# jmhb0/view_neti

Measured on AMD Instinct MI355X. Metric: TI train steps/sec (SD-1.5 512^2 bs=4 per GPU), higher is better.
Workload: dtype f16; 1 GPU; learnable_mode 0, sd15 shapes, 512x512 fp16, bs=4/GPU, grad_accum 1, full train step (VAE+16xCLIP+UNet fwd/bwd+AdamW); global_batch=4, parallelism=dp1, rccl_ranks=1, hipgraph=True

## Files before the change

include/vneti.h:

```cpp
#ifndef VNETI_H
#define VNETI_H
#include <stddef.h>
#include <stdint.h>

#ifdef __cplusplus
extern "C" {
#endif

#define VNETI_ABI_VERSION 1

int vneti_version(void);
int vneti_precision(void);
int vneti_last_error(char* buf, size_t n);

typedef struct vneti_gemm_desc {
  const void* A;
  const void* B;
  void* C;
  long long lda, ldb, ldc;
  int M, N, K;
  int batch;
  long long strideA, strideB, strideC;
  const float* bias;
  const void* rowadd;
  long long ld_rowadd;
  int rows_per_group;
  const void* resid;
  long long ldr;
  float alpha;
  int act;
  int out_f32;
  int conv_mode;
  int Hi, Wi, Ci, Ho, Wo, stride, pad_t, pad_l, ups;
  long long ldx;
  int tile_hint;
  void* workspace;
  long long workspace_bytes;
  int split_k;
  const void* gate_src;
  long long ld_gate;
  int gate_act;
  void* C2;
  long long ldc2;
  int act2;
  void* gn_sums;
  int gn_hw, gn_cpg, gn_groups, gn_slots;
  int geglu;
  int conv_korder;
} vneti_gemm_desc;

int vneti_gemm_f16(const vneti_gemm_desc* d, void* stream);
int vneti_gemm_select_tile(int M, int N, int batch);
int vneti_gemm_select_split(int M, int N, int K, int batch, int tile_hint, long long workspace_bytes);

int vneti_im2col3x3_small(const void* x, int x_is_f32, long long sb, long long sc, long long sy,
                          long long sx, void* out, int Bn, int C, int Hi, int Wi, int Ho, int Wo,
                          int stride, int pad_t, int pad_l, void* stream);

int vneti_conv3x3_in(const void* x, int x_is_f32, long long sb, long long sc, long long sy, long long sx,
                     const void* w_packed, const float* bias, void* out, long long ldo, int Bn, int C, int H, int W,
                     int Co, void* gn_sums, int gn_groups, int gn_slots, void* stream);

int vneti_transpose_f16(const void* in, long long ld_in, long long stride_in, void* out,
                        long long ld_out, long long stride_out, int rows, int cols, int batch,
                        void* stream);
#define VNETI_TRANSPOSE_MAX 4
typedef struct vneti_transpose_desc {
  const void* inp;
  long long ld_in, stride_in;
  void* out;
  long long ld_out, stride_out;
  int rows, cols, batch, _pad;
} vneti_transpose_desc;
int vneti_transpose_f16_multi(const vneti_transpose_desc* descs, int n, void* stream);

long long vneti_groupnorm_ws_floats(int Bn, int HW, int C, int G);
int vneti_groupnorm_fwd(const void* x, long long ldx, void* y, long long ldy, const float* gamma,
                        const float* beta, float* mean, float* rstd, float* ws, int Bn, int HW,
                        int C, int G, float eps, int silu, void* stream);
int vneti_groupnorm_fwd_sums(const void* x, long long ldx, void* y, long long ldy, const float* gamma,
                             const float* beta, const void* sums, int slots, float* mean, float* rstd,
// ... 220 lines not shown
```

view_neti_amd/csrc/gemm8.hip:

```cpp
#include <type_traits>

#include "common.h"
#include "gemm_args.h"

namespace {

constexpr int BM = 256, NT = 512;
constexpr int HALF_BYTES = 128 * 128;
constexpr int GN_IMG = 5;

#define VN_WAIT_VM(n) asm volatile("s_waitcnt vmcnt(" #n ")" ::: "memory")
#define VN_WAIT_LGKM0() asm volatile("s_waitcnt lgkmcnt(0)" ::: "memory")

template <int BN, int EPI, bool CONV, bool HALO = false>
__global__ __launch_bounds__(NT) void gemm8_kernel(GemmArgs g) {
  static_assert(BN == 256 || BN == 128, "tile width");
  static_assert(!HALO || (BN == 128 && CONV), "the halo-patch loop exists for the 256x128 convolution tile");
  constexpr int PATCH_STRIDE = 41 * 1024;
  constexpr bool H42 = HALO && BN == 128;
  constexpr int NJB = BN / 128;
  constexpr int HB_BYTES = (BN / 2) * 128;
  constexpr int HB_DMA = BN / 128;
  constexpr int NBUF = BN == 256 ? 2 : 3;
  constexpr int BUF_BYTES = 2 * HALF_BYTES + 2 * HB_BYTES;
// ... 41 lines not shown
  auto rowmem = [&](const int r) { return HALO ? row0 + (r >> 4) * g.Wo + (r & 15) : m0 + r; };

  const half_t* Ab = g.A + (long long)bz * g.strideA;
  const half_t* Bb = g.B + (long long)bz * g.strideB;
  const __amdgpu_buffer_rsrc_t rsA = vn_make_rsrc(Ab, g.a_bytes);
  const __amdgpu_buffer_rsrc_t rsB = vn_make_rsrc(Bb, g.b_bytes);

  const int lrow = tid >> 3;
  const int gchunk = (tid & 7) ^ ((lrow >> 1) & 7);
  const float rcp_hw = CONV ? 1.0f / (float)(g.Ho * g.Wo) : 0.f, rcp_wo = CONV ? 1.0f / (float)g.Wo : 0.f;
  int a_base[4];
  uint32_t a_mask[4];
#pragma unroll
  for (int r = 0; r < (HALO ? 0 : 4); ++r) {
    const int m = m0 + (r >> 1) * 128 + (r & 1) * 64 + lrow;
    const bool ok = m < g.M;
    if constexpr (!CONV) {
      a_base[r] = (int)((long long)m * g.lda * 2) + gchunk * 16;
      a_mask[r] = ok ? 1u : 0u;
    } else {
      const int hw = g.Ho * g.Wo;
      int b = (int)((float)m * rcp_hw);
      int rem = m - b * hw;
      if (rem < 0) { b -= 1; rem += hw; } else if (rem >= hw) { b += 1; rem -= hw; }
      int oy = (int)((float)rem * rcp_wo);
      int ox = rem - oy * g.Wo;
      if (ox < 0) { oy -= 1; ox += g.Wo; } else if (ox >= g.Wo) { oy += 1; ox -= g.Wo; }
      const int py = e_conv == 1 ? oy * g.stride - g.pad_t : oy + g.pad_t;
      const int px = e_conv == 1 ? ox * g.stride - g.pad_l : ox + g.pad_l;
      a_base[r] = ((b * g.Hi + py) * g.Wi + px) * g.ldx2 + gchunk * 16;
      const int sgn = e_conv == 1 ? 1 : -1;
      uint32_t colbits = 0, mask = 0;
#pragma unroll
      for (int d = 0; d < 3; ++d) colbits |= ((unsigned)(px + sgn * d) < (unsigned)g.Wi ? 1u : 0u) << d;
#pragma unroll
      for (int d = 0; d < 3; ++d) mask |= ((unsigned)(py + sgn * d) < (unsigned)g.Hi ? colbits : 0u) << (3 * d);
      a_mask[r] = ok ? mask : 0u;
    }
  }
  uint32_t b_base[4];
#pragma unroll
  for (int r = 0; r < 4; ++r) {
    const int n = n0 + (r >> 1) * (BN / 2) + (r & 1) * 64 + lrow;
    b_base[r] = (n < g.N) ? (uint32_t)((long long)n * g.ldb * 2) + gchunk * 16 : VN_OOB;
  }

  const int nk_total = g.K / 64;
  const int kt_begin = kz * g.kt_per_split;
  const int kt_end = min(nk_total, kt_begin + g.kt_per_split);
  const int T = kt_end - kt_begin;

  int a_kt[2] = {kt_begin, kt_begin}, b_kt[2] = {kt_begin, kt_begin};
  int a_tap[2], a_ci0[2];
  {
    int tap = 0, ci0 = 0;
    if constexpr (CONV) {
      if (g.korder) {
        ci0 = (kt_begin / 9) * 64;
        tap = kt_begin - (kt_begin / 9) * 9;
      } else {
        tap = (kt_begin * 64) / g.Ci;
        ci0 = kt_begin * 64 - tap * g.Ci;
      }
    }
    a_tap[0] = a_tap[1] = tap;
    a_ci0[0] = a_ci0[1] = ci0;
  }
  const int tap_step = (e_conv == 2 ? -1 : 1) * g.ldx2;
  uint32_t nxt[4];
  auto prepA = [&](const int h) {
    const bool live = a_kt[h] < kt_end;
    int soff;
    uint32_t tapbit;
    if constexpr (!CONV) {
      soff = a_kt[h] * 128;
      tapbit = live ? 1u : 0u;
    } else {
      const int tap = a_tap[h];
      const int dy = (tap * 11) >> 5;
      const int dx = tap - 3 * dy;
      soff = (dy * g.Wi + dx) * tap_step + a_ci0[h] * 2;
      tapbit = live ? (1u << tap) : 0u;
      if (g.korder) {
        a_tap[h] += 1;
        if (a_tap[h] == 9) {
          a_tap[h] = 0;
          a_ci0[h] += 64;
        }
      } else {
        a_ci0[h] += 64;
        if (a_ci0[h] == g.Ci) {
          a_ci0[h] = 0;
          a_tap[h] += 1;
        }
      }
    }
#pragma unroll
    for (int j = 0; j < 2; ++j) {
      nxt[j] = (a_mask[2 * h + j] & tapbit) ? (uint32_t)(a_base[2 * h + j] + soff) : VN_OOB;
    }
    a_kt[h] += 1;
  };
  auto prepB = [&](const int h) {
    const bool live = b_kt[h] < kt_end;
    const uint32_t soff = (uint32_t)b_kt[h] * 128u, dead = live ? 0u : VN_OOB;
    if constexpr (BN == 256) {
#pragma unroll
      for (int j = 0; j < 2; ++j) nxt[j] = (b_base[2 * h + j] + soff) | dead;
    } else {
      nxt[2 + h] = (b_base[2 * h] + soff) | dead;
    }
    b_kt[h] += 1;
  };
// ... 673 lines not shown
```

view_neti_amd/csrc/gemm_args.h:

```cpp
#pragma once
#include "common.h"

namespace {

struct GemmArgs {
  const half_t* A;
  const half_t* B;
  void* C;
  const float* bias;
  const half_t* rowadd;
  const void* resid;
  float* ws;
  const half_t* gate_src;
  half_t* C2;
  long long ld_gate, ldc2;
  int gate_act, act2;
  float* gn_sums;
  int gn_hw, gn_cpg, gn_G, gn_slots;
  int geglu;
  long long lda, ldb, ldc, ld_rowadd, ldr;
  long long strideA, strideB, strideC;
  uint32_t a_bytes, b_bytes;
  int M, N, K;
  int rows_per_group;
  float alpha;
  int act;
  int out_f32;
  int batch, ksplit, kt_per_split;
  int conv_mode;
  int Hi, Wi, Ci, Ho, Wo, stride, pad_t, pad_l, ups;
  int ldx2;
  int korder;
  int tiles_m, tiles_n;
};

__device__ __forceinline__ float apply_act(float v, int act) {
  switch (act) {
    case 1: return vn_silu(v);
    case 2: return vn_quick_gelu(v);
    case 3: return vn_gelu_erf(v);
    default: return v;
  }
}
__device__ __forceinline__ float act_grad(float f, int act) {
  if (act == 2) {
    float s = vn_sigmoid(1.702f * f);
    return s * (1.f + 1.702f * f * (1.f - s));
  } else if (act == 3) {
    return vn_gelu_erf_grad(f);
  }
  float s = vn_sigmoid(f);
  return s * (1.f + f * (1.f - s));
}

__device__ __forceinline__ int lds_off(int row, int chunk) {
  return row * 128 + ((chunk ^ ((row >> 1) & 7)) << 4);
}

__device__ __forceinline__ void dma16(__amdgpu_buffer_rsrc_t rs, char* lds_dst, uint32_t off) {
#if defined(__HIP_DEVICE_COMPILE__)
  __builtin_amdgcn_raw_ptr_buffer_load_lds(rs, (__attribute__((address_space(3))) void*)lds_dst, 16, off, 0, 0, 0);
#else
  (void)rs; (void)lds_dst; (void)off;
#endif
}

}
// ... 3 lines not shown
```

view_neti_amd/csrc/gemm_conv.hip:

```cpp
#include "common.h"
#include "gemm_args.h"
#include "../../include/vneti.h"

namespace {

template <int BM, int BN, int WM, int WN, bool F32OUT, bool DMA, int NSTG = 2, int EPI = 2, bool CONV = true>
__global__ __launch_bounds__((BM / WM) * (BN / WN) * 64) void gemm_kernel(
    const half_t* pA, const half_t* pB, uint32_t p_a_bytes, uint32_t p_b_bytes, int p_lda, int p_ldb, int pM, int pN, int pK,
    int p_tiles_m, int p_tiles_n, int p_split_conv , const GemmArgs gfull) {
  GemmArgs g = gfull;
  g.A = pA;
  g.B = pB;
  g.a_bytes = p_a_bytes;
  g.b_bytes = p_b_bytes;
  g.lda = p_lda;
  g.ldb = p_ldb;
  g.M = pM;
  g.N = pN;
  g.K = pK;
  g.tiles_m = p_tiles_m;
  g.tiles_n = p_tiles_n;
  g.kt_per_split = p_split_conv & 0xffff;
  g.ksplit = (p_split_conv >> 16) & 0xff;
  g.conv_mode = p_split_conv >> 24;
// ... 99 lines not shown
      if (g.stride == 2) {
        ok = ok && ((ty | tx) & 1) == 0;
        ty >>= 1;
        tx >>= 1;
      }
      iy = ty;
      ix = tx;
      ok = ok && iy < g.Hi && ix < g.Wi;
    }
    return ok ? (uint32_t)(((a_bh[i] + iy) * g.Wi + ix) * g.ldx2 + tapoff) : VN_OOB;
  };

  uint32_t a_cur[A_IT], b_cur[B_IT];
#pragma unroll
  for (int i = 0; i < B_IT; ++i) b_cur[i] = b_off[i] < 0 ? VN_OOB : (uint32_t)b_off[i];

  auto issue = [&](int kt, int stage, bool first) {
    const int k0 = kt * 64;
    bool recompute = first;
    int dy = 0, dx = 0, tapoff = 0;
    if (e_conv != 0) {
      int tap, ci0;
      if (g.korder) {
        const int chunk = kt / 9;
        tap = kt - chunk * 9;
        ci0 = chunk << 6;
        recompute = true;
      } else {
        tap = k0 / g.Ci;
        ci0 = k0 - tap * g.Ci;
        recompute = recompute || ci0 == 0;
      }
      if (recompute) {
        dy = tap / 3;
        dx = tap - dy * 3;
        tapoff = (e_conv == 1 && !g.ups) ? ((dy * g.Wi + dx) * g.ldx2 + ci0 * 2) : (ci0 * 2 + gchunk * 16);
      }
    }
    if (recompute) {
#pragma unroll
      for (int i = 0; i < A_IT; ++i) a_cur[i] = a_offset(i, k0, dy, dx, tapoff);
      if (first) {
#pragma unroll
        for (int i = 0; i < B_IT; ++i) b_cur[i] += (uint32_t)k0 * 2;
      }
    }
    if constexpr (DMA) {
      char* As = smem + stage * STAGE_BYTES;
      char* Bs = As + BM * 128;
#pragma unroll
      for (int i = 0; i < A_IT; ++i) dma16(rsA, As + (wave * 8 + RSTEP * i) * 128, a_cur[i]);
#pragma unroll
      for (int i = 0; i < B_IT; ++i) dma16(rsB, Bs + (wave * 8 + RSTEP * i) * 128, b_cur[i]);
    } else {
#pragma unroll
      for (int i = 0; i < A_IT; ++i) ra[i] = vn_buf_load16(rsA, a_cur[i]);
#pragma unroll
      for (int i = 0; i < B_IT; ++i) rb[i] = vn_buf_load16(rsB, b_cur[i]);
    }
#pragma unroll
    for (int i = 0; i < A_IT; ++i) a_cur[i] += 128;
#pragma unroll
    for (int i = 0; i < B_IT; ++i) b_cur[i] += 128;
  };

  auto store_lds = [&](int stage) {
    if constexpr (!DMA) {
      char* As = smem + stage * STAGE_BYTES;
// ... 579 lines not shown
  g.C2 = (half_t*)d->C2;
  g.ldc2 = d->ldc2;
  g.act2 = d->act2;
  g.gn_sums = (float*)d->gn_sums;
  g.gn_hw = d->gn_hw;
  g.gn_cpg = d->gn_cpg;
  g.gn_G = d->gn_groups;
  g.gn_slots = d->gn_slots;
  g.geglu = d->geglu;
  g.lda = d->lda;
  g.ldb = d->ldb;
  g.ldc = d->ldc;
  g.ld_rowadd = d->ld_rowadd;
  g.ldr = d->ldr;
  g.strideA = d->strideA;
  g.strideB = d->strideB;
  g.strideC = d->strideC;
  g.M = d->M;
  g.N = d->N;
  g.K = d->K;
  g.batch = batch;
  g.rows_per_group = d->rows_per_group > 0 ? d->rows_per_group : 1;
  g.alpha = d->alpha;
  g.act = d->act;
  g.out_f32 = d->out_f32 ? 1 : 0;
  g.conv_mode = d->conv_mode;
  long long a_bytes;
  if (d->conv_mode == 0) {
    VN_REQUIRE(d->lda % 8 == 0, "gemm: lda=%lld must be a multiple of 8", d->lda);
    a_bytes = ((long long)(d->M - 1) * d->lda + d->K) * 2;
  } else {
    VN_REQUIRE(d->conv_mode == 1 || d->conv_mode == 2, "gemm: bad conv_mode %d", d->conv_mode);
    VN_REQUIRE(d->Ci > 0 && d->Ci % 64 == 0, "conv: Ci=%d must be a multiple of 64", d->Ci);
    VN_REQUIRE(d->K == 9 * d->Ci, "conv: K=%d must equal 9*Ci=%d", d->K, 9 * d->Ci);
    VN_REQUIRE(d->stride == 1 || d->stride == 2, "conv: stride %d unsupported", d->stride);
    VN_REQUIRE(d->Ho > 0 && d->Wo > 0 && d->M % (d->Ho * d->Wo) == 0, "conv: M=%d not a multiple of Ho*Wo", d->M);
    VN_REQUIRE(d->ldx % 8 == 0, "conv: ldx must be a multiple of 8");
    VN_REQUIRE(!(d->ups && d->conv_mode != 1), "conv: fused upsample only in forward gather mode");
    VN_REQUIRE(!(d->ups && d->stride != 1), "conv: fused upsample needs stride 1");
    g.Hi = d->Hi;
    g.Wi = d->Wi;
    g.Ci = d->Ci;
    g.Ho = d->Ho;
    g.Wo = d->Wo;
    g.stride = d->stride;
    g.pad_t = d->pad_t;
    g.pad_l = d->pad_l;
    g.ups = d->ups;
    g.ldx2 = (int)(d->ldx * 2);
    VN_REQUIRE(!d->conv_korder || d->Ci % 64 == 0, "conv: conv_korder=1 needs Ci=%d to be a multiple of 64", d->Ci);
    g.korder = d->conv_korder ? 1 : 0;
    long long nb = d->M / (d->Ho * d->Wo);
    a_bytes = nb * d->Hi * d->Wi * d->ldx * 2;
  }
  long long b_bytes = ((long long)(d->N - 1) * d->ldb + d->K) * 2;
  VN_REQUIRE(a_bytes < 0x7fffffffLL && b_bytes < 0x7fffffffLL, "gemm: operand larger than 2 GiB");
  g.a_bytes = (uint32_t)a_bytes;
  g.b_bytes = (uint32_t)b_bytes;
  if (!d->out_f32) {
    VN_REQUIRE(d->ldc % 8 == 0 || d->N < 8, "gemm: ldc=%lld must be a multiple of 8", d->ldc);
  }
  VN_REQUIRE_OUT("gemm C", vn_out_bytes(d->M, d->ldc, d->N, d->out_f32 ? 4 : 2, batch, d->strideC));
  if (d->C2) VN_REQUIRE_OUT("gemm C2", vn_out_bytes(d->M, d->ldc2, d->geglu == 1 ? d->N / 2 : d->N, 2));
  hipStream_t st = (hipStream_t)stream;
  bool f32 = d->out_f32 != 0;
  VN_REQUIRE(!(f32 && d->rowadd), "gemm: rowadd is only supported for f16 output");
  if (d->gate_src || d->C2) {
// ... 2 lines not shown
    VN_REQUIRE(!d->C2 || (d->act2 >= 0 && d->act2 <= 3 && d->ldc2 % 8 == 0), "gemm: bad C2 arguments");
  }

  if (d->geglu) {
    VN_REQUIRE(d->geglu == 1 || d->geglu == 2, "gemm: geglu must be 0, 1 or 2");
    VN_REQUIRE(!f32 && batch == 1 && d->N % 8 == 0, "gemm: geglu needs f16 output, batch 1 and N %% 8 == 0");
    VN_REQUIRE(d->split_k == 1, "gemm: geglu needs split_k = 1 (it lives in the fused epilogue)");
    VN_REQUIRE(!d->gn_sums, "gemm: geglu and gn_sums are exclusive");
    if (d->geglu == 1) {
      VN_REQUIRE(d->C2 && d->ldc2 % 4 == 0 && !d->gate_src, "gemm: geglu forward needs C2 ([M][N/2]) and no gate");
    } else {
      VN_REQUIRE(d->gate_src && d->ld_gate % 8 == 0 && !d->C2 && !d->resid && !d->rowadd,
                 "gemm: geglu backward needs gate_src ([M][2N] saved pre-activation) and a plain epilogue");
      VN_REQUIRE(d->ldc % 8 == 0, "gemm: geglu backward writes [M][2N]: ldc %% 8");
    }
  }
  if (d->gn_sums) {
    VN_REQUIRE(!f32 && batch == 1, "gemm: gn_sums needs f16 output and batch 1");
    VN_REQUIRE(d->gn_hw >= 64 && d->gn_cpg >= 4 && d->gn_groups > 0 && d->gn_slots > 0 && d->N == d->gn_cpg * d->gn_groups &&
                   d->M % d->gn_hw == 0 && (d->gn_cpg >= 8 || d->gn_cpg == 4),
               "gemm: bad gn_sums geometry hw=%d cpg=%d G=%d", d->gn_hw, d->gn_cpg, d->gn_groups);
    VN_REQUIRE(d->split_k == 1, "gemm: gn_sums needs split_k = 1 (the statistics live in the fused epilogue)");
  }

  int cfg = d->tile_hint;
  bool dma = true;
  if (cfg >= 100) {
    dma = false;
    cfg -= 100;
  }
  if (cfg == 0) cfg = select_tile(d->M, d->N, batch);
  VN_REQUIRE(cfg >= 1 && cfg <= kMaxTile, "gemm: unknown tile_hint %d", d->tile_hint);
  if (cfg == 18 &&
      (d->conv_mode < 1 || d->conv_mode > 2 || d->stride != 1 || d->ups || d->pad_t != 1 || d->pad_l != 1 || d->Hi != d->Ho ||
       d->Wi != d->Wo || (d->Ho & 15) || (d->Wo & 15) || (d->Ci & 63) || !d->conv_korder || batch != 1 || f32))
    cfg = 17;
  if (cfg == 18 && d->gn_sums && (d->gn_cpg & 1)) cfg = 17;
  if ((cfg == 16 || cfg == 17) && (!dma || (d->conv_mode && (d->ups || (d->conv_mode == 2 && d->stride == 2))) ||
                    (d->gn_sums && (d->gn_cpg & 1)) ||
                    (d->M >= (1 << 24) && (d->conv_mode || d->rowadd || d->gn_sums)))) cfg = cfg == 16 ? 5 : 7;
  if ((cfg == 5 || cfg == 16) && f32) cfg = 4;
  if (cfg == 17 && f32) cfg = 7;
  if ((cfg == 6 || cfg == 7) && !dma) cfg = 4;
  if (cfg >= 10 && !dma) cfg = kTiles[cfg].bm == 128 ? (kTiles[cfg].bn == 128 ? 1 : 2) : 3;
  long long ws_floats = d->workspace ? d->workspace_bytes / 4 : 0;
  int ks = d->split_k;
  if (ks == 0) ks = select_ksplit(d->M, d->N, d->K, batch, cfg, ws_floats);
  if (ks < 1) ks = 1;
  const int nk = d->K / 64;
  if (ks > nk) ks = nk;
  if (ks > 1) {
    VN_REQUIRE(d->workspace && (long long)ks * batch * d->M * d->N <= ws_floats,
               "gemm: split_k=%d needs %lld workspace bytes", ks, (long long)ks * batch * d->M * d->N * 4);
    VN_REQUIRE(batch == 1 || (d->strideC != 0), "gemm: batched split-K needs strideC");
    VN_REQUIRE((long long)batch * d->M * ((d->N + 3) / 4) < 0x7fffffffLL, "gemm: split-K output larger than 2^31 chunks");
    VN_REQUIRE_OUT("gemm split-K workspace", (long long)ks * batch * d->M * d->N * 4);
  }
  if (cfg == 18 && ks > d->Ci / 64) ks = d->Ci / 64;
  g.ksplit = ks;
  g.kt_per_split = cdiv(nk, ks);
  g.ksplit = cdiv(nk, g.kt_per_split);
  VN_REQUIRE(g.ksplit <= 255 && g.kt_per_split <= 0xffff, "gemm: split_k=%d / K=%d out of range", g.ksplit, d->K);
  g.ws = (float*)d->workspace;

#define LAUNCH(BM, BN, WM, WN) \
  return dma ? launch_cfg<BM, BN, WM, WN, true>(g, f32, st) : launch_cfg<BM, BN, WM, WN, false>(g, f32, st)
  switch (cfg) {
// ... 28 lines not shown
```

view_neti_amd/engine/schedule.py:

```python
from __future__ import annotations

from functools import partial
from typing import Dict, List

import torch

from .. import lib, ops, packing


class T:

    __slots__ = ("v", "g", "gw", "rows", "cols", "children", "need_grad", "producer")

    def __init__(self, v, g=None, need_grad=True):
        self.v = v
        self.g = g
        self.gw = False
        self.rows, self.cols = v.shape
        self.children: List["T"] = []
        self.need_grad = need_grad
        self.producer = None


def rup(x, m):
# ... 64 lines not shown
            t.gw = True
            for c in t.children:
                c.gw = True

    @staticmethod
    def _tagged(p, fn):
        if hasattr(fn, "vn_cost"):
            p.vn_cost = fn.vn_cost
        return p

    def _contrib_gemm(self, t: T, A, Bm, **kw):
        g = self._grad(t)
        resid = g if t.gw else None
        self.bwd.append(partial(ops.gemm, A, Bm, g, resid=resid, **kw))
        if not t.gw:
            t.gw = True
            for c in t.children:
                c.gw = True

    _tile_cache: Dict[tuple, int] = {}
    _TILE_DIMS = {1: (128, 128), 2: (128, 64), 3: (64, 64), 4: (256, 128), 5: (256, 256), 6: (256, 128), 7: (256, 128),
                  8: (256, 128), 9: (128, 128), 10: (128, 128), 11: (128, 64), 12: (64, 64), 13: (128, 128), 14: (128, 64),
                  15: (64, 64), 16: (256, 256), 17: (256, 128), 18: (256, 128)}

    @staticmethod
    def _gemm_key(f):
        kw = f.keywords
        A, Bm, out = f.args[:3]
        conv = kw.get("conv")
        M = kw.get("M") or A.shape[-2]
        N = kw.get("N") or Bm.shape[-2]
        K = kw.get("K") or Bm.shape[-1]
        ck = (conv["mode"], conv["stride"], conv["ups"], conv["Hi"], conv["Wi"]) if conv else None
        return (M, N, K, kw.get("batch") or 1, ck, out.dtype == torch.float32, kw.get("geglu") or 0)

    def autotune(self, candidates=(1, 2, 3, 5, 6, 7, 8, 9, 10, 11, 12, 13, 14, 15, 16, 17, 18), reps=8):
        if not torch.cuda.is_available():
            return
        import json
        import os
        from .. import parallel
        if os.environ.get("VNETI_AUTOTUNE_CANDS"):
            candidates = tuple(int(x) for x in os.environ["VNETI_AUTOTUNE_CANDS"].split(","))
        how = _timing_switches(self.dev, reps)
        cache = Schedule._tile_cache
        cache_path = os.environ.get("VNETI_AUTOTUNE_CACHE")
        if cache_path and os.path.exists(cache_path) and not cache:
            cache.update(picks_from_json(json.load(open(cache_path))))
        n_before = len(cache)
        share = parallel.sharing_picks() and parallel._dist() is not None
        rank0 = (not share) or parallel._dist().get_rank() == 0
        if share and not rank0:
            cache.update(parallel.share_from_rank0(None))
        for lst in (self.fwd_pre, self.fwd, self.bwd):
            for idx, f in enumerate(lst):
                if getattr(f, "func", None) is not ops.gemm or f.keywords.get("tile_hint"):
                    continue
                key = self._gemm_key(f)
                B_cm = None
                if key not in cache:
                    cache[key], B_cm = self._measure(f, key, candidates, how)
                lst[idx] = self._pin(f, cache[key], B_cm)
        if share and rank0:
            parallel.share_from_rank0(dict(cache))
        if cache_path and len(cache) != n_before and parallel.world_info()[0] == 0:
            tmp = f"{cache_path}.{os.getpid()}.tmp"
            with open(tmp, "w") as fh:
                json.dump(picks_to_json(cache), fh)
            os.replace(tmp, cache_path)

    def _measure(self, f, key, candidates, how):
        conv = f.keywords.get("conv")
        B_cm = packing._chunk_major(f.args[1], f.args[1].shape[0], conv["Ci"]) if _chunk_major_ok(conv) else None
        best, best_t = (0, 0, 0), float("inf")
        for h, sk, ko in gemm_variants(key, conv, f.keywords.get("geglu"), candidates):
            kw = dict(f.keywords)
            kw["tile_hint"], kw["split_k"] = h, sk
            args = f.args
            if ko:
                kw["conv"] = dict(conv, korder=1)
                args = (f.args[0], B_cm) + tuple(f.args[2:])
            t = _time_call(partial(ops.gemm, *args, **kw), args[0], *how)
            if t < best_t:
                best, best_t = (h, sk, ko), t
        return best, B_cm

    def _pin(self, f, pick, B_cm=None):
        pick = tuple(pick) + (0,) * (3 - len(pick))
        conv = f.keywords.get("conv")
        kw = dict(f.keywords)
        kw["tile_hint"], kw["split_k"] = pick[0], pick[1]
        args = f.args
        if pick[2] and _chunk_major_ok(conv):
            if B_cm is None:
                B_cm = packing._chunk_major(f.args[1], f.args[1].shape[0], conv["Ci"])
            kw["conv"] = dict(conv, korder=1)
            self.bytes += B_cm.numel() * B_cm.element_size()
            args = (f.args[0], B_cm) + tuple(f.args[2:])
        return partial(ops.gemm, *args, **kw)

    def bind_workspace(self):
        for lst in (self.fwd_pre, self.fwd, self.bwd):
            for idx, f in enumerate(lst):
                fn = getattr(f, "func", None)
                if fn is ops.gemm or fn is ops.attn_bwd_dkv:
                    lst[idx] = self._rebound(f, fn, dict(f.keywords, workspace=self.ws))

    @staticmethod
    def _rebound(f, fn, kw):
        return partial(fn, *f.args, **kw)

    GN_SLOTS = 8

    def _produced(self, t: T):
        t.producer = len(self.fwd) - 1
        return t

    GN2_MAX = 512

    def _gn2_slice(self):
        if not hasattr(self, "_gn2_arena"):
            self._gn2_arena = self._buf((self.GN2_MAX, self.B, self.GN_SLOTS, self.groups, 4), torch.int64, zero=True)
            self._gn2_used = 0
        assert self._gn2_used < self.GN2_MAX
        self._gn2_used += 1
        return self._gn2_arena[self._gn2_used - 1]

    def fuse_gn_stats(self, fuse: bool = True):
        n = self._fuse_gn_stats() if fuse else 0
        if getattr(self, "_gn2_used", 0):
            self.fwd.insert(0, self._gn2_arena[:self._gn2_used].zero_)
        return n

    def _fuse_gn_stats(self):
        import os
        if os.environ.get("VNETI_NO_GN_FUSE"):
            return 0
        S, G, B = self.GN_SLOTS, self.groups, self.B
# ... 45 lines not shown
                   rstd=self._buf((self.B * self.groups,), torch.float32), silu=silu, hw=hw)
        y = self._buf((x.rows, Cc))
        import os
        if os.environ.get("VNETI_GN_3L"):
            self.fwd.append(partial(ops.groupnorm_fwd, x.v, y, rec["gamma"], rec["beta"], rec["mean"], rec["rstd"],
                                    self.gn_ws, self.B, hw, Cc, self.groups, eps, silu))
        else:
            self.fwd.append(partial(ops.groupnorm_fwd_2l, x.v, y, rec["gamma"], rec["beta"], self._gn2_slice(),
                                    self.GN_SLOTS, rec["mean"], rec["rstd"], self.B, hw, Cc, self.groups, eps, silu))
            if self.need_backward:
                rec["bsums"] = self._gn2_slice()
        if x.producer is not None:
            self._gn_fusable.append(dict(idx=len(self.fwd) - 1, prod=x.producer, gn=rec, x=x.v, y=y, hw=hw, C=Cc,
                                         eps=eps, silu=silu))
        return y, rec

    def _gn_bwd_fn(self, rec, dy):
        x = rec["x"]
        if "bsums" not in rec:
            fn = lambda out, accum: ops.groupnorm_bwd(dy, x.v, rec["gamma"], rec["beta"], rec["mean"], rec["rstd"], out,
                                                      self.gn_ws, self.B, rec["hw"], x.cols, self.groups,
                                                      rec["silu"], accum=accum)
        else:
            fn = lambda out, accum: ops.groupnorm_bwd_2l(dy, x.v, rec["gamma"], rec["beta"], rec["mean"], rec["rstd"], out,
                                                         rec["bsums"], self.GN_SLOTS, self.gn_ws, self.B, rec["hw"], x.cols,
                                                         self.groups, rec["silu"], accum=accum)
        fn.vn_cost = ("GroupNorm(+SiLU) bwd", 5.0 * self.B * rec["hw"] * x.cols * 2)
        return fn

    def _conv_desc(self, Hi, Wi, Ci, Ho, Wo, stride, pad, ups, ldx, mode=1):
        return dict(mode=mode, Hi=Hi, Wi=Wi, Ci=Ci, Ho=Ho, Wo=Wo, stride=stride, pad_t=pad, pad_l=pad, ups=ups,
                    ldx=ldx, korder=1 if (packing.KORDER_CM and Ci % 64 == 0) else 0)

    def _resnet(self, x: T, cin, cout, name, w, out_view, h, wd, need_dx=True):
        M = x.rows
        n1, gn1 = self._gn(x, name + "norm1", w, self.eps, True)
        w1 = self._w16(packing.conv3x3_fwd(w[name + "conv1.weight"]))
        b1 = self._w32(w[name + "conv1.bias"])
        radd = None
        if name in self.temb_off:
            off, n = self.temb_off[name]
            radd = self.temb_all[:, off:off + n]
        h1 = T(self._buf((M, cout)))
        self.fwd.append(partial(ops.gemm, n1, w1, h1.v, bias=b1, rowadd=radd, rows_per_group=h * wd, M=M,
                                conv=self._conv_desc(h, wd, cin, h, wd, 1, 1, 0, cin)))
        self._produced(h1)
        n2, gn2 = self._gn(h1, name + "norm2", w, self.eps, True)
        w2 = self._w16(packing.conv3x3_fwd(w[name + "conv2.weight"]))
        b2 = self._w32(w[name + "conv2.bias"])
        out = T(out_view if out_view is not None else self._buf((M, cout)))
        wsc = None
        if cin != cout:
            wsc = self._w16(w[name + "conv_shortcut.weight"].reshape(cout, cin))
            bsc = self._w32(w[name + "conv_shortcut.bias"])
            sc_buf = self._buf((M, cout))
            self.fwd.append(partial(ops.gemm, x.v, wsc, sc_buf, bias=bsc))
            resid = sc_buf
        else:
            resid = x.v
        self.fwd.append(partial(ops.gemm, n2, w2, out.v, bias=b2, resid=resid, M=M,
                                conv=self._conv_desc(h, wd, cout, h, wd, 1, 1, 0, cout)))
        self._produced(out)
        rec = dict(kind="resnet", x=x, out=out, h1=h1, gn1=gn1, gn2=gn2, cin=cin, cout=cout, h=h, wd=wd,
                   need_dx=need_dx, name=name)
        if self.need_backward and need_dx:
            rec["w2d"] = self._w16(packing.conv3x3_dgrad(w[name + "conv2.weight"]))
# ... 42 lines not shown
        out = T(out_view if out_view is not None else self._buf((M, Cc)))
        self.fwd.append(partial(ops.gemm, x.v, wf, out.v, bias=b, M=M,
                                conv=self._conv_desc(h, wd, Cc, h // 2, wd // 2, 2, pad, 0, x.v.stride(0))))
        self._produced(out)
        rec = dict(kind="down", x=x, out=out, C=Cc, h=h, wd=wd, pad=pad)
        if self.need_backward:
            rec["wd_"] = self._w16(packing.conv3x3_dgrad(w[name + "weight"]))
        self.tape.append(rec)
        return out

    def _downsample_bwd(self, r):
        x, out, Cc, h, wd = r["x"], r["out"], r["C"], r["h"], r["wd"]
        assert out.gw
        desc = self._conv_desc(h // 2, wd // 2, Cc, h, wd, 2, r["pad"], 0, out.g.stride(0), mode=2)
        self._contrib_gemm(x, out.g, r["wd_"], M=x.rows, conv=desc)

    def forward_pre(self):
        for f in self.fwd_pre:
            f()

    def forward_main(self):
        for f in self.fwd:
            f()

    def forward(self):
        self.forward_pre()
        self.forward_main()

    def backward(self):
        for f in self.bwd:
            f()


def _chunk_major_ok(conv) -> bool:
    return bool(conv) and not conv.get("ups") and not conv.get("korder") and \
        not (conv["mode"] == 2 and conv["stride"] == 2) and conv["Ci"] % 64 == 0 and conv["Ci"] >= 128


def gemm_variants(key, conv, geglu, candidates) -> List[tuple]:
    M, N, K, batch = key[:4]
    try_cm = _chunk_major_ok(conv)
    halo_ok = try_cm and conv["mode"] in (1, 2) and conv["stride"] == 1 and conv["pad_t"] == 1 and conv["pad_l"] == 1 \
        and conv["Ho"] % 16 == 0 and conv["Wo"] % 16 == 0 and conv["Hi"] == conv["Ho"] and conv["Wi"] == conv["Wo"]
    tiles_ko = [(h, 0) for h in candidates if h != 18] + \
        ([(h, 1) for h in candidates if h in (16, 17) or (h == 18 and halo_ok)] if try_cm else [])
    out = []
    for h, ko in tiles_ko:
        bm, bn = Schedule._TILE_DIMS[h]
        tiles = -(-M // bm) * -(-N // bn) * batch
        sks = (0, 1) + (tuple(x for x in (2, 3, 4, 6, 8, 12)
                              if x * 8 <= K // 64 and tiles * x <= 1024 and x * batch * M * N <= 16 * 2 ** 20)
                        if tiles < 256 else ())
        if geglu:
            sks = (1,)
        out += [(h, sk, ko) for sk in sks]
    return out


def _timing_switches(dev, reps):
    import os
    cold = None if os.environ.get("VNETI_AUTOTUNE_HOT") else torch.empty(160 * 2 ** 20, dtype=torch.float32, device=dev)
    return (cold, reps, int(os.environ.get("VNETI_AUTOTUNE_REPS", "9")),
            bool(int(os.environ.get("VNETI_AUTOTUNE_WARM_A", "1"))))


def _time_call(call, act, cold, reps, cold_reps, warm_a):
    call()
    call()
# ... 42 lines not shown
```

view_neti_amd/engine/unet.py:

```python
from __future__ import annotations

from functools import partial
from typing import Dict

import torch

from .. import ops, packing
from .. import sd_config as sc
from .schedule import Schedule, T, rup as _rup


class UNetEngine(Schedule):
    def __init__(self, cfg: sc.UNetConfig, weights: Dict[str, torch.Tensor], batch: int, height: int, width: int,
                 ctx_len: int = 77, device: str = "cuda", need_backward: bool = True, autotune: bool = True,
                 fuse_gn: bool = True):
        super().__init__(batch, cfg.norm_num_groups, cfg.norm_eps, device, need_backward)
        self.cfg = cfg
        self.H, self.W = height, width
        self.L = ctx_len
        self.nl = cfg.n_cross_layers
        B, L, Dc = batch, ctx_len, cfg.cross_attention_dim
        self.x_in = self._buf((B, cfg.in_channels, height, width), torch.float32)
        self.timesteps = torch.zeros(B, dtype=torch.int64, device=device)
        self.ctx_k = self._buf((self.nl, B * L, Dc))
        self.ctx_v = self._buf((self.nl, B * L, Dc))
        self.dctx_k = self._buf((self.nl, B * L, Dc))
        self.dctx_v = self._buf((self.nl, B * L, Dc))
        self.pred = self._buf((B * height * width, 8))[:, : cfg.out_channels]
        self.dpred = self._buf((B * height * width, 8), zero=True)[:, : cfg.out_channels]
        self._pack_time_weights(weights)
        self._plan_kv()
        self._build(weights)
        self._kv_fwd_ops()
        if need_backward:
            self._build_backward()
            self._kv_bwd_ops()
        if autotune:
            self.autotune()
        self.bind_workspace()
        self.fuse_gn_stats(fuse=fuse_gn)
# ... 181 lines not shown
            return
        dn2 = self._tmp("tA", M, Cc)
        bw.append(partial(ops.gemm, dq2, r["wq2d"], dn2))
        dh1 = self._tmp("tF", M, Cc)
        bw.append(partial(self._ln_bwd, r["ln2"], dn2, dh1, dh2))
        do1 = self._tmp("tA", M, Cc)
        bw.append(partial(ops.gemm, dh1, r["wo1d"], do1))
        qkv = r["qkv"]
        q, k, v = qkv[:, :Cc], qkv[:, Cc:2 * Cc], qkv[:, 2 * Cc:]
        dqkv = self._tmp("tC", M, 3 * Cc)
        dq, dk, dv = dqkv[:, :Cc], dqkv[:, Cc:2 * Cc], dqkv[:, 2 * Cc:]
        bw.append(partial(ops.attn_bwd_dq, q, k, v, do1, r["lse1"], delta, dq, B, heads, N, N, D, r["scale"], False,
                          O=r["o1"]))
        bw.append(partial(ops.attn_bwd_dkv, q, k, v, do1, r["lse1"], delta, dk, dv, B, heads, N, N, D, r["scale"],
                          False))
        dn1 = self._tmp("tD", M, Cc)
        bw.append(partial(ops.gemm, dqkv, r["wqkvd"], dn1))
        dh0 = self._tmp("tE", M, Cc)
        bw.append(partial(self._ln_bwd, r["ln1"], dn1, dh0, dh1))
        dg = self._tmp("tA", M, Cc)
        bw.append(partial(ops.gemm, dh0, r["w_ind"], dg))
        self._contrib(x, self._gn_bwd_fn(r["gn"], dg), extra=dout)

    def _upsample(self, x: T, Cc, name, w, out_view, h, wd):
        M = x.rows * 4
        wf = self._w16(packing.conv3x3_fwd(w[name + "weight"]))
        b = self._w32(w[name + "bias"])
        out = T(out_view if out_view is not None else self._buf((M, Cc)))
        self.fwd.append(partial(ops.gemm, x.v, wf, out.v, bias=b, M=M,
                                conv=self._conv_desc(h, wd, Cc, 2 * h, 2 * wd, 1, 1, 1, x.v.stride(0))))
        self._produced(out)
        rec = dict(kind="up", x=x, out=out, C=Cc, h=h, wd=wd)
        if self.need_backward:
            rec["wd_"] = self._w16(packing.conv3x3_dgrad(w[name + "weight"]))
        self.tape.append(rec)
        return out

    def _upsample_bwd(self, r):
        x, out, Cc, h, wd = r["x"], r["out"], r["C"], r["h"], r["wd"]
        assert out.gw and not x.gw
        M = out.rows
        dup = self._tmp("dA", M, Cc)
        self.bwd.append(partial(ops.gemm, out.g, r["wd_"], dup, M=M,
                                conv=self._conv_desc(2 * h, 2 * wd, Cc, 2 * h, 2 * wd, 1, 1, 0, out.g.stride(0), mode=2)))
        g = self._grad(x)
        self.bwd.append(partial(ops.sum2x2, dup, g, self.B, h, wd, Cc))
        x.gw = True

    def _build(self, w):
        cfg = self.cfg
        B, H, W = self.B, self.H, self.W
        boc = cfg.block_out_channels
        nlev = len(boc)
        nres = cfg.layers_per_block + 1
        self._time_ops()
        catT = {}
        for i in range(nlev):
            lvl = nlev - 1 - i
            m = B * (H >> lvl) * (W >> lvl)
            for j in range(nres):
                rin, skip, _ = sc.up_block_channels(cfg, i, j)
                catT[(i, j)] = T(self._buf((m, rin + skip)),
                                 self._buf((m, rin + skip)) if self.need_backward else None)

        def h_slot(key):
            rin = sc.up_block_channels(cfg, *key)[0]
            return catT[key].v[:, :rin]

        def adopt(t: T, key, part):
            rin = sc.up_block_channels(cfg, *key)[0]
            cat = catT[key]
            if cat.g is not None:
                t.g = cat.g[:, :rin] if part == "h" else cat.g[:, rin:]
            cat.children.append(t)
# ... 113 lines not shown
```

view_neti_amd/ops.py:

```python
from __future__ import annotations

import ctypes as C

import torch

from . import lib as _l

ACT_NONE, ACT_SILU, ACT_QUICK_GELU, ACT_GELU = 0, 1, 2, 3


def stream() -> int:
    return torch.cuda.current_stream().cuda_stream


def _p(t):
    return None if t is None else t.data_ptr()


def _ld(t):
    if t is None:
        return 0
    assert t.stride(-1) == 1, "last dim must be contiguous"
    return t.stride(-2) if t.dim() >= 2 else t.shape[-1]


_default_ws = None


def set_default_gemm_workspace(t):
    global _default_ws
    _default_ws = t


def gemm(A, B, out, *, bias=None, rowadd=None, rows_per_group=1, resid=None, alpha=1.0, act=0,
         tile_hint=0, batch=0, strideA=0, strideB=0, strideC=0, M=None, N=None, K=None, conv=None,
         lda=None, ldc=None, workspace=None, split_k=0, gate=None, gate_act=0, out2=None, act2=0,
         gn_sums=None, gn_hw=0, gn_groups=0, gn_slots=0, geglu=0):
    d = _l.GemmDesc()
    d.A, d.B, d.C = _p(A), _p(B), _p(out)
    d.ldb = _ld(B)
    d.ldc = ldc if ldc is not None else _ld(out)
    d.N = N if N is not None else B.shape[-2]
    d.K = K if K is not None else B.shape[-1]
    if conv is None:
        d.M = M if M is not None else A.shape[-2]
        d.lda = lda if lda is not None else _ld(A)
        d.conv_mode = 0
    else:
        d.M = M
        d.lda = 0
        d.conv_mode = conv["mode"]
        for k in ("Hi", "Wi", "Ci", "Ho", "Wo", "stride", "pad_t", "pad_l", "ups", "ldx"):
            setattr(d, k, int(conv.get(k, 0)))
        d.conv_korder = int(conv.get("korder", 0))
    d.batch = batch
    d.strideA, d.strideB, d.strideC = strideA, strideB, strideC
    d.bias = _p(bias)
    d.rowadd = _p(rowadd)
    d.ld_rowadd = _ld(rowadd) if rowadd is not None else 0
    d.rows_per_group = rows_per_group
    d.resid = _p(resid)
    d.ldr = _ld(resid) if resid is not None else 0
    d.alpha = alpha
    d.act = act
    d.out_f32 = 1 if out.dtype == torch.float32 else 0
    d.tile_hint = tile_hint
    if gate is not None:
        d.gate_src, d.ld_gate, d.gate_act = _p(gate), _ld(gate), gate_act
    if out2 is not None:
        d.C2, d.ldc2, d.act2 = _p(out2), _ld(out2), act2
    if gn_sums is not None:
        d.gn_sums, d.gn_hw, d.gn_groups, d.gn_slots = _p(gn_sums), gn_hw, gn_groups, gn_slots
        d.gn_cpg = d.N // gn_groups
    d.geglu = geglu
    ws = workspace if workspace is not None else _default_ws
    if ws is not None:
        d.workspace = ws.data_ptr()
        d.workspace_bytes = ws.numel() * ws.element_size()
    d.split_k = split_k if ws is not None else 1
    _l.call("gemm_f16", C.byref(d), stream())


def im2col3x3_small(x, out, Bn, Cc, Hi, Wi, Ho, Wo, stride, pad_t, pad_l, strides):
    sb, sc, sy, sx = strides
    _l.call("im2col3x3_small", _p(x), 1 if x.dtype == torch.float32 else 0, sb, sc, sy, sx, _p(out),
            Bn, Cc, Hi, Wi, Ho, Wo, stride, pad_t, pad_l, stream())


def conv3x3_in(x, w_packed, bias, out, Bn, Cc, H, W, strides, gn_sums=None, gn_hw=0, gn_groups=0, gn_slots=0):
    sb, sc, sy, sx = strides
    assert gn_sums is None or gn_hw == H * W
    _l.call("conv3x3_in", _p(x), 1 if x.dtype == torch.float32 else 0, sb, sc, sy, sx, _p(w_packed), _p(bias), _p(out),
            _ld(out), Bn, Cc, H, W, w_packed.shape[0], _p(gn_sums), gn_groups, gn_slots, stream())


def transpose(inp, out, rows, cols, batch, ld_in, stride_in, ld_out, stride_out):
    _l.call("transpose_f16", _p(inp), ld_in, stride_in, _p(out), ld_out, stride_out, rows, cols, batch, stream())


def transpose_multi(items):
    arr = (_l.TransposeDesc * len(items))()
    for d, (inp, out, rows, cols, batch, ld_in, stride_in, ld_out, stride_out) in zip(arr, items):
        d.inp, d.ld_in, d.stride_in = _p(inp), ld_in, stride_in
        d.out, d.ld_out, d.stride_out = _p(out), ld_out, stride_out
        d.rows, d.cols, d.batch = rows, cols, batch
    _l.call("transpose_f16_multi", arr, len(items), stream())


def groupnorm_ws_floats(Bn, HW, Cc, G):
    n = _l.query("groupnorm_ws_floats", Bn, HW, Cc, G)
    if n < 0:
        raise RuntimeError(f"groupnorm: unsupported shape {(Bn, HW, Cc, G)}")
    return n


# ... 465 lines not shown
```

view_neti_amd/packing.py:

```python
from __future__ import annotations

import os

import torch

KORDER_CM = os.environ.get("VNETI_CONV_KORDER", "0") == "1"


def _chunk_major(m: torch.Tensor, n_out: int, c: int) -> torch.Tensor:
    return m.reshape(n_out, 9, c // 64, 64).permute(0, 2, 1, 3).reshape(n_out, 9 * c).contiguous()


def conv3x3_fwd(w: torch.Tensor, cm=None) -> torch.Tensor:
    co, ci, kh, kw = w.shape
    assert kh == 3 and kw == 3
    m = w.permute(0, 2, 3, 1).reshape(co, 9 * ci).contiguous()
    cm = KORDER_CM if cm is None else cm
    return _chunk_major(m, co, ci) if cm and ci % 64 == 0 else m


def conv3x3_dgrad(w: torch.Tensor, cm=None) -> torch.Tensor:
    co, ci, kh, kw = w.shape
    assert kh == 3 and kw == 3
    m = w.permute(1, 2, 3, 0).reshape(ci, 9 * co).contiguous()
    cm = KORDER_CM if cm is None else cm
    return _chunk_major(m, ci, co) if cm and co % 64 == 0 else m


def pad_rows(w: torch.Tensor, mult: int) -> torch.Tensor:
    k = w.shape[-1]
    kp = (k + mult - 1) // mult * mult
    if kp == k:
        return w.contiguous()
    out = torch.zeros(*w.shape[:-1], kp, dtype=w.dtype, device=w.device)
    out[..., :k] = w
    return out


def geglu_interleave_index(n2: int, device=None) -> torch.Tensor:
    F = n2 // 2
    assert n2 % 8 == 0
    r = torch.arange(n2, device=device)
    q, e = r // 8, r % 8
    return torch.where(e < 4, 4 * q + e, F + 4 * q + e - 4)


def geglu_interleave(w: torch.Tensor) -> torch.Tensor:
    return w[geglu_interleave_index(w.shape[0], w.device)].contiguous()


def conv_in_direct(w: torch.Tensor) -> torch.Tensor:
    co, ci, kh, kw = w.shape
    assert kh == 3 and kw == 3 and 9 * ci <= 32 and co % 128 == 0
    m = torch.zeros(co, 32, dtype=w.dtype)
    m[:, : 9 * ci] = w.permute(0, 2, 3, 1).reshape(co, 9 * ci)
    j = torch.arange(8).view(8, 1, 1)
    fq = torch.arange(4).view(1, 4, 1)
    e = torch.arange(4).view(1, 1, 4)
    src = ((j // 2) * 32 + fq * 8 + (j % 2) * 4 + e).reshape(128)
# ... 3 lines not shown
```

view_neti_amd/roofline.py:

```python
from __future__ import annotations

import torch

from . import ops

import os as _os

_CSRC = _os.path.join(_os.path.dirname(_os.path.abspath(__file__)), "csrc")
MFMA_PEAK_TFLOPS = 2500.0
HBM_PEAK_TBS = 8.0
PF, TB = MFMA_PEAK_TFLOPS, HBM_PEAK_TBS


def kernel_tree_sha() -> str:
    import hashlib
    import os
    here = _CSRC
    files = sorted(os.path.join(here, f) for f in os.listdir(here) if f.endswith((".hip", ".h")))
    files.append(os.path.join(os.path.dirname(os.path.dirname(here)), "include", "vneti.h"))
    h = hashlib.sha256()
    for f in files:
        h.update(os.path.basename(f).encode())
        h.update(open(f, "rb").read())
    return h.hexdigest()[:16]


def gemm_cost(f):
    kw = f.keywords
    A, Bm = f.args[0], f.args[1]
    M = kw.get("M") or A.shape[-2]
    N, K = kw.get("N") or Bm.shape[-2], kw.get("K") or Bm.shape[-1]
    batch = kw.get("batch") or 1
    conv = kw.get("conv")
    a_bytes = (M // (conv["Ho"] * conv["Wo"])) * conv["Hi"] * conv["Wi"] * conv["Ci"] * 2 if conv else M * K * 2 * batch
    out = f.args[2]
    c_cols = N * (2 if kw.get("geglu") == 2 else 1)
    extra = sum(M * c * 2 for c, key in ((N, "resid"), (N, "out2"), (c_cols, "gate")) if kw.get(key) is not None)
    if kw.get("geglu") == 1:
        extra -= M * N
    nbytes = a_bytes + N * K * 2 * batch + M * c_cols * out.element_size() * batch + extra
    flops = 2.0 * M * N * K * batch
    return M, N, K, batch, flops, nbytes, flops / (MFMA_PEAK_TFLOPS * 1e12), nbytes / (HBM_PEAK_TBS * 1e12)



def cost(f):
    fn, a, kw = getattr(f, "func", None), getattr(f, "args", ()), getattr(f, "keywords", {}) or {}
    if fn is ops.gemm:
        M, N, K, batch, flops, nbytes, t_mfma, t_hbm = gemm_cost(f)
        if t_hbm > t_mfma:
            return ("gemm, below the ridge (short-K linears: HBM-bound)", 0, nbytes)
        return ("gemm / implicit-GEMM conv (MFMA-bound)", flops, 0)
    if fn in (ops.attn_fwd, ops.attn_bwd_dq, ops.attn_bwd_dkv):
        i = {ops.attn_fwd: 5, ops.attn_bwd_dq: 7, ops.attn_bwd_dkv: 8}[fn]
        Bn, H, Nq, Nk, D = a[i:i + 5]
        causal = a[i + 6]
        mm = {ops.attn_fwd: 2, ops.attn_bwd_dq: 3, ops.attn_bwd_dkv: 4}[fn]
        name = {ops.attn_fwd: "attention fwd", ops.attn_bwd_dq: "attention bwd dQ", ops.attn_bwd_dkv: "attention bwd dK/dV"}[fn]
        scores = Bn * H * Nq * Nk * (0.5 if causal else 1.0)
        ks, db = -(-D // 16), -(-D // 32)
        mfma_c = {ops.attn_fwd: ks + 2 * db, ops.attn_bwd_dq: 2 * ks + 2 * db, ops.attn_bwd_dkv: 2 * ks + 4 * db}[fn] * 32 / 1024.0
        valu_c = {ops.attn_fwd: 2.8, ops.attn_bwd_dq: 4.0, ops.attn_bwd_dkv: 4.0}[fn] * 2 / 64.0 + (2 * 5 / 3) / 64.0
        cob = scores * (mfma_c + valu_c) / (1024 * 2.4e9)
        return (name, mm * 2.0 * scores * D, 0, cob)
    if fn is ops.attn_bwd_small:
        Bn, H, N, D = a[9:13]
        return ("attention bwd (short sequences, one launch)", 7 * 2.0 * Bn * H * N * N * D * (0.5 if a[14] else 1.0), 0)
    if fn in (ops.groupnorm_fwd, ops.groupnorm_fwd_sums, ops.groupnorm_fwd_2l):
        Bn, HW, C = (a[7], a[8], a[9]) if fn is ops.groupnorm_fwd else (a[8], a[9], a[10])
        return ("GroupNorm(+SiLU) fwd" + (" (stats in producer)" if fn is ops.groupnorm_fwd_sums else ""), 0, 2.0 * Bn * HW * C * 2)
    if fn is ops.layernorm_fwd:
        x, y = a[0], a[1]
        return ("LayerNorm fwd", 0, x.numel() * x.element_size() + y.numel() * y.element_size())
    if getattr(f, "vn_cost", None) is not None:
        return (f.vn_cost[0], 0, f.vn_cost[1])
    if getattr(fn, "__name__", "") == "_ln_bwd":
        x = a[0]["x"]
        n = x.numel()
        extra = (a[3].numel() * a[3].element_size() if a[3] is not None else 0) + (n * 2 if len(a) > 4 and a[4] is not None else 0)
        return ("LayerNorm bwd", 0, n * x.element_size() + a[1].numel() * a[1].element_size() + a[2].numel() * a[2].element_size() + extra)
    if fn in (ops.groupnorm_bwd, ops.groupnorm_bwd_2l):
# ... 75 lines not shown
```

Before: 40.03 steps/s.

## Fold nearest-upsample into a 4x4 stride-2 conv for upsampler dgrad

The backward of upsample+3x3 conv previously ran a full-resolution 3x3 transposed conv into a temporary followed by a 2x2 sum. This folds the nearest-upsample into precomputed summed 4x4 weights and computes the input gradient directly as a stride-2 4x4 conv at low resolution. The GEMM conv gather is generalized to KHxKW windows up to 4x4. That cuts MACs and drops the temporary and the sum pass, at the cost of a new weight packing, restrictions on tile config 18, and extra per-tap divide arithmetic in the kernel.

```diff
diff --git a/include/vneti.h b/include/vneti.h
--- a/include/vneti.h
+++ b/include/vneti.h
@@ -47,6 +47,7 @@
   int gn_hw, gn_cpg, gn_groups, gn_slots;
   int geglu;
   int conv_korder;
+  int conv_kh, conv_kw;
 } vneti_gemm_desc;
 
 int vneti_gemm_f16(const vneti_gemm_desc* d, void* stream);
diff --git a/view_neti_amd/csrc/gemm8.hip b/view_neti_amd/csrc/gemm8.hip
--- a/view_neti_amd/csrc/gemm8.hip
+++ b/view_neti_amd/csrc/gemm8.hip
@@ -97,9 +97,9 @@
       const int sgn = e_conv == 1 ? 1 : -1;
       uint32_t colbits = 0, mask = 0;
 #pragma unroll
-      for (int d = 0; d < 3; ++d) colbits |= ((unsigned)(px + sgn * d) < (unsigned)g.Wi ? 1u : 0u) << d;
-#pragma unroll
-      for (int d = 0; d < 3; ++d) mask |= ((unsigned)(py + sgn * d) < (unsigned)g.Hi ? colbits : 0u) << (3 * d);
+      for (int d = 0; d < 4; ++d) colbits |= (d < g.KW && (unsigned)(px + sgn * d) < (unsigned)g.Wi ? 1u : 0u) << d;
+#pragma unroll
+      for (int d = 0; d < 4; ++d) mask |= (d < g.KH && (unsigned)(py + sgn * d) < (unsigned)g.Hi ? colbits : 0u) << (g.KW * d);
       a_mask[r] = ok ? mask : 0u;
     }
   }
@@ -142,8 +142,8 @@
       tapbit = live ? 1u : 0u;
     } else {
       const int tap = a_tap[h];
-      const int dy = (tap * 11) >> 5;
-      const int dx = tap - 3 * dy;
+      const int dy = (tap * g.kw_mul) >> 8;
+      const int dx = tap - g.KW * dy;
       soff = (dy * g.Wi + dx) * tap_step + a_ci0[h] * 2;
       tapbit = live ? (1u << tap) : 0u;
       if (g.korder) {
diff --git a/view_neti_amd/csrc/gemm_args.h b/view_neti_amd/csrc/gemm_args.h
--- a/view_neti_amd/csrc/gemm_args.h
+++ b/view_neti_amd/csrc/gemm_args.h
@@ -32,7 +32,11 @@
   int ldx2;
   int korder;
   int tiles_m, tiles_n;
+  int KH, KW;
+  int kw_mul;
 };
+
+inline int vn_kw_mul(int kw) { return (256 + kw - 1) / kw; }
 
 __device__ __forceinline__ float apply_act(float v, int act) {
   switch (act) {
diff --git a/view_neti_amd/csrc/gemm_conv.hip b/view_neti_amd/csrc/gemm_conv.hip
--- a/view_neti_amd/csrc/gemm_conv.hip
+++ b/view_neti_amd/csrc/gemm_conv.hip
@@ -155,8 +155,8 @@
         recompute = recompute || ci0 == 0;
       }
       if (recompute) {
-        dy = tap / 3;
-        dx = tap - dy * 3;
+        dy = (tap * g.kw_mul) >> 8;
+        dx = tap - dy * g.KW;
         tapoff = (e_conv == 1 && !g.ups) ? ((dy * g.Wi + dx) * g.ldx2 + ci0 * 2) : (ci0 * 2 + gchunk * 16);
       }
     }
@@ -802,7 +802,14 @@
   } else {
     VN_REQUIRE(d->conv_mode == 1 || d->conv_mode == 2, "gemm: bad conv_mode %d", d->conv_mode);
     VN_REQUIRE(d->Ci > 0 && d->Ci % 64 == 0, "conv: Ci=%d must be a multiple of 64", d->Ci);
-    VN_REQUIRE(d->K == 9 * d->Ci, "conv: K=%d must equal 9*Ci=%d", d->K, 9 * d->Ci);
+    const int kh = d->conv_kh ? d->conv_kh : 3, kw = d->conv_kw ? d->conv_kw : 3;
+    VN_REQUIRE(kh >= 1 && kh <= 4 && kw >= 1 && kw <= 4, "conv: window %d x %d out of range (1..4 each)", kh, kw);
+    VN_REQUIRE((kh == 3 && kw == 3) || (d->conv_mode == 1 && !d->ups && !d->conv_korder),
+               "conv: a %d x %d window needs the plain forward gather (conv_mode 1, no ups) in tap-major K order", kh, kw);
+    VN_REQUIRE(d->K == kh * kw * d->Ci, "conv: K=%d must equal %d*Ci=%d", d->K, kh * kw, kh * kw * d->Ci);
+    g.KH = kh;
+    g.KW = kw;
+    g.kw_mul = vn_kw_mul(kw);
     VN_REQUIRE(d->stride == 1 || d->stride == 2, "conv: stride %d unsupported", d->stride);
     VN_REQUIRE(d->Ho > 0 && d->Wo > 0 && d->M % (d->Ho * d->Wo) == 0, "conv: M=%d not a multiple of Ho*Wo", d->M);
     VN_REQUIRE(d->ldx % 8 == 0, "conv: ldx must be a multiple of 8");
@@ -871,7 +878,7 @@
   if (cfg == 0) cfg = select_tile(d->M, d->N, batch);
   VN_REQUIRE(cfg >= 1 && cfg <= kMaxTile, "gemm: unknown tile_hint %d", d->tile_hint);
   if (cfg == 18 &&
-      (d->conv_mode < 1 || d->conv_mode > 2 || d->stride != 1 || d->ups || d->pad_t != 1 || d->pad_l != 1 || d->Hi != d->Ho ||
+      (d->conv_mode < 1 || d->conv_mode > 2 || g.KH != 3 || g.KW != 3 || d->stride != 1 || d->ups || d->pad_t != 1 || d->pad_l != 1 || d->Hi != d->Ho ||
        d->Wi != d->Wo || (d->Ho & 15) || (d->Wo & 15) || (d->Ci & 63) || !d->conv_korder || batch != 1 || f32))
     cfg = 17;
   if (cfg == 18 && d->gn_sums && (d->gn_cpg & 1)) cfg = 17;
diff --git a/view_neti_amd/engine/schedule.py b/view_neti_amd/engine/schedule.py
--- a/view_neti_amd/engine/schedule.py
+++ b/view_neti_amd/engine/schedule.py
@@ -120,6 +120,8 @@
         N = kw.get("N") or Bm.shape[-2]
         K = kw.get("K") or Bm.shape[-1]
         ck = (conv["mode"], conv["stride"], conv["ups"], conv["Hi"], conv["Wi"]) if conv else None
+        if conv and _window(conv) != (3, 3):
+            ck += _window(conv)
         return (M, N, K, kw.get("batch") or 1, ck, out.dtype == torch.float32, kw.get("geglu") or 0)
 
     def autotune(self, candidates=(1, 2, 3, 5, 6, 7, 8, 9, 10, 11, 12, 13, 14, 15, 16, 17, 18), reps=8):
@@ -142,7 +144,7 @@
             cache.update(parallel.share_from_rank0(None))
         for lst in (self.fwd_pre, self.fwd, self.bwd):
             for idx, f in enumerate(lst):
-                if getattr(f, "func", None) is not ops.gemm or f.keywords.get("tile_hint"):
+                if getattr(f, "func", None) not in ops.GEMM_LAUNCHES or f.keywords.get("tile_hint"):
                     continue
                 key = self._gemm_key(f)
                 B_cm = None
@@ -185,13 +187,13 @@
             kw["conv"] = dict(conv, korder=1)
             self.bytes += B_cm.numel() * B_cm.element_size()
             args = (f.args[0], B_cm) + tuple(f.args[2:])
-        return partial(ops.gemm, *args, **kw)
+        return partial(f.func, *args, **kw)
 
     def bind_workspace(self):
         for lst in (self.fwd_pre, self.fwd, self.bwd):
             for idx, f in enumerate(lst):
                 fn = getattr(f, "func", None)
-                if fn is ops.gemm or fn is ops.attn_bwd_dkv:
+                if fn in ops.GEMM_LAUNCHES or fn is ops.attn_bwd_dkv:
                     lst[idx] = self._rebound(f, fn, dict(f.keywords, workspace=self.ws))
 
     @staticmethod
@@ -303,6 +305,9 @@
         return dict(mode=mode, Hi=Hi, Wi=Wi, Ci=Ci, Ho=Ho, Wo=Wo, stride=stride, pad_t=pad, pad_l=pad, ups=ups,
                     ldx=ldx, korder=1 if (packing.KORDER_CM and Ci % 64 == 0) else 0)
 
+    def _conv4x4s2_desc(self, Hi, Wi, Ci, ldx):
+        return dict(self._conv_desc(Hi, Wi, Ci, Hi // 2, Wi // 2, 2, 1, 0, ldx), korder=0, kh=4, kw=4)
+
     def _resnet(self, x: T, cin, cout, name, w, out_view, h, wd, need_dx=True):
         M = x.rows
         n1, gn1 = self._gn(x, name + "norm1", w, self.eps, True)
@@ -411,8 +416,12 @@
             f()
 
 
+def _window(conv) -> tuple:
+    return (conv.get("kh") or 3, conv.get("kw") or 3)
+
+
 def _chunk_major_ok(conv) -> bool:
-    return bool(conv) and not conv.get("ups") and not conv.get("korder") and \
+    return bool(conv) and not conv.get("ups") and not conv.get("korder") and _window(conv) == (3, 3) and \
         not (conv["mode"] == 2 and conv["stride"] == 2) and conv["Ci"] % 64 == 0 and conv["Ci"] >= 128
 
 
diff --git a/view_neti_amd/engine/unet.py b/view_neti_amd/engine/unet.py
--- a/view_neti_amd/engine/unet.py
+++ b/view_neti_amd/engine/unet.py
@@ -5,7 +5,7 @@
 
 import torch
 
-from .. import ops, packing
+from .. import lib, ops, packing
 from .. import sd_config as sc
 from .schedule import Schedule, T, rup as _rup
 
@@ -253,7 +253,10 @@
         self._produced(out)
         rec = dict(kind="up", x=x, out=out, C=Cc, h=h, wd=wd)
         if self.need_backward:
-            rec["wd_"] = self._w16(packing.conv3x3_dgrad(w[name + "weight"]))
+            if Cc % 64 == 0:
+                rec["wd4"] = self._w16(packing.upsample_dgrad4x4(w[name + "weight"], lib.act_dtype()))
+            else:
+                rec["wd_"] = self._w16(packing.conv3x3_dgrad(w[name + "weight"]))
         self.tape.append(rec)
         return out
 
@@ -261,6 +264,11 @@
         x, out, Cc, h, wd = r["x"], r["out"], r["C"], r["h"], r["wd"]
         assert out.gw and not x.gw
         M = out.rows
+        if "wd4" in r:
+            self.bwd.append(partial(ops.upsample_dgrad, out.g, r["wd4"], self._grad(x), M=x.rows,
+                                    conv=self._conv4x4s2_desc(2 * h, 2 * wd, Cc, out.g.stride(0))))
+            x.gw = True
+            return
         dup = self._tmp("dA", M, Cc)
         self.bwd.append(partial(ops.gemm, out.g, r["wd_"], dup, M=M,
                                 conv=self._conv_desc(2 * h, 2 * wd, Cc, 2 * h, 2 * wd, 1, 1, 0, out.g.stride(0), mode=2)))
diff --git a/view_neti_amd/ops.py b/view_neti_amd/ops.py
--- a/view_neti_amd/ops.py
+++ b/view_neti_amd/ops.py
@@ -53,6 +53,7 @@
         for k in ("Hi", "Wi", "Ci", "Ho", "Wo", "stride", "pad_t", "pad_l", "ups", "ldx"):
             setattr(d, k, int(conv.get(k, 0)))
         d.conv_korder = int(conv.get("korder", 0))
+        d.conv_kh, d.conv_kw = int(conv.get("kh", 0)), int(conv.get("kw", 0))
     d.batch = batch
     d.strideA, d.strideB, d.strideC = strideA, strideB, strideC
     d.bias = _p(bias)
@@ -81,6 +82,15 @@
     _l.call("gemm_f16", C.byref(d), stream())
 
 
+def upsample_dgrad(dy, w4, out, **kw):
+    conv = kw["conv"]
+    assert (conv["mode"], conv["stride"], conv.get("kh"), conv.get("kw"), conv.get("ups") or 0) == (1, 2, 4, 4, 0)
+    gemm(dy, w4, out, **kw)
+
+
+GEMM_LAUNCHES = (gemm, upsample_dgrad)
+
+
 def im2col3x3_small(x, out, Bn, Cc, Hi, Wi, Ho, Wo, stride, pad_t, pad_l, strides):
     sb, sc, sy, sx = strides
     _l.call("im2col3x3_small", _p(x), 1 if x.dtype == torch.float32 else 0, sb, sc, sy, sx, _p(out),
diff --git a/view_neti_amd/packing.py b/view_neti_amd/packing.py
--- a/view_neti_amd/packing.py
+++ b/view_neti_amd/packing.py
@@ -25,6 +25,23 @@
     m = w.permute(1, 2, 3, 0).reshape(ci, 9 * co).contiguous()
     cm = KORDER_CM if cm is None else cm
     return _chunk_major(m, ci, co) if cm and co % 64 == 0 else m
+
+
+_UPS_DGRAD_TAPS = ((2,), (1, 2), (0, 1), (0,))
+
+
+def upsample_dgrad4x4(w: torch.Tensor, dtype=None) -> torch.Tensor:
+    co, ci, kh, kw = w.shape
+    assert kh == 3 and kw == 3
+    wr = w if dtype is None else w.to(dtype)
+    wr = wr.to(torch.float64 if w.dtype == torch.float64 else torch.float32)
+    m = wr.new_zeros(ci, 4, 4, co)
+    for u, ty in enumerate(_UPS_DGRAD_TAPS):
+        for v, tx in enumerate(_UPS_DGRAD_TAPS):
+            for dy in ty:
+                for dx in tx:
+                    m[:, u, v, :] += wr[:, :, dy, dx].t()
+    return m.reshape(ci, 16 * co)
 
 
 def pad_rows(w: torch.Tensor, mult: int) -> torch.Tensor:
diff --git a/view_neti_amd/roofline.py b/view_neti_amd/roofline.py
--- a/view_neti_amd/roofline.py
+++ b/view_neti_amd/roofline.py
@@ -46,7 +46,7 @@
 
 def cost(f):
     fn, a, kw = getattr(f, "func", None), getattr(f, "args", ()), getattr(f, "keywords", {}) or {}
-    if fn is ops.gemm:
+    if fn in ops.GEMM_LAUNCHES:
         M, N, K, batch, flops, nbytes, t_mfma, t_hbm = gemm_cost(f)
         if t_hbm > t_mfma:
             return ("gemm, below the ridge (short-K linears: HBM-bound)", 0, nbytes)
```

Result: no change. 40.27 steps/s, median of 6 (+0.6%).
